# xiph/flac

Measured on NVIDIA H100. Metric: encode_msamples_per_s, higher is better.
Workload: dtype int32

## Files before the change

### flac_b200/csrc/autoc_kernel.cuh

```cuda
#pragma once

#include "device_common.cuh"

namespace fb200 {

__device__ __forceinline__ void cp_async_16(void *smem, const void *gmem)
{
	const unsigned s = (unsigned)__cvta_generic_to_shared(smem);
	asm volatile("cp.async.cg.shared.global [%0], [%1], 16;\n" ::"r"(s), "l"(gmem) : "memory");
}
__device__ __forceinline__ void cp_async_4_zfill(void *smem, const void *gmem, int src_bytes)
{
	const unsigned s = (unsigned)__cvta_generic_to_shared(smem);
	asm volatile("cp.async.ca.shared.global [%0], [%1], 4, %2;\n" ::"r"(s), "l"(gmem), "r"(src_bytes) : "memory");
}
__device__ __forceinline__ void cp_async_commit() { asm volatile("cp.async.commit_group;\n" ::: "memory"); }
template <int N>
__device__ __forceinline__ void cp_async_wait() { asm volatile("cp.async.wait_group %0;\n" ::"n"(N) : "memory"); }

__host__ __device__ constexpr int autoc3_stride(int T) { return ((T / 4) % 2 == 1) ? T : T + 4; }
template <int LAGS, int U, int K, int STAGES>
constexpr size_t autoc3_smem_bytes() { return (size_t)STAGES * (32 * autoc3_stride(U * K) + U * K) * 4; }

template <int LAGS, int U, int K, int STAGES>
__global__ void __launch_bounds__(32) k_autoc3(EncK P, const int32_t *__restrict__ sig, const SigMeta *__restrict__ meta,
                                              const float *__restrict__ windows, const DevSection *__restrict__ secs,
                                              double *__restrict__ autoc, int nitems)
{
	static_assert(U % LAGS == 0 && U % 4 == 0, "a body must be a whole number of history rotations and of 128-bit loads");
	constexpr int T = U * K;
	constexpr int STRIDE = autoc3_stride(T);
	constexpr int STAGE_WORDS = 32 * STRIDE + T;
	extern __shared__ int4 autoc3_smem[];
	int *const smem = reinterpret_cast<int *>(autoc3_smem);

	const int lane = threadIdx.x;
	const int groups = (nitems + 31) >> 5;
	const int sec = blockIdx.x / groups;
	const int item0 = (blockIdx.x - sec * groups) << 5;
	const int item = item0 + lane;
	const bool live = item < nitems && meta[min(item, nitems - 1)].bps != 0;
	if(!__any_sync(0xffffffffu, live)) return;

	const DevSection S = secs[sec];
	const float *w = windows + S.win_off;
	const int shift = S.partial ? S.data_shift : 0;
	const int a0 = shift & ~3;
	const int nvalid = S.partial ? 2 * S.part_size : S.data_len;
	const int wsecond = P.bs - 2 * S.part_size;
	const int ntiles = (shift - a0 + nvalid + T - 1) / T;

	auto issue = [&](int t) {
		if(t < ntiles) {
			int *st = smem + (t % STAGES) * STAGE_WORDS;
			const int32_t *g0 = sig + a0 + t * T;
#pragma unroll
			for(int j = 0; j < T / 4; j++) {
				const int idx = j * 32 + lane;
				const int row = idx / (T / 4), c = idx - row * (T / 4);
				cp_async_16(st + row * STRIDE + c * 4, g0 + (size_t)min(item0 + row, nitems - 1) * P.bs_stride + c * 4);
			}
#pragma unroll
			for(int j = 0; j < (T + 31) / 32; j++) {
				const int u = j * 32 + lane;
				if(u < T) {
					const int i = a0 + t * T + u - shift;
					const bool ok = i >= 0 && i < nvalid;
					const int wi = (!S.partial || i < S.part_size) ? i : wsecond + i;
					cp_async_4_zfill(st + 32 * STRIDE + u, ok ? (w + wi) : w, ok ? 4 : 0);
				}
			}
		}
		cp_async_commit();
	};

	double acc[LAGS], h[LAGS];
#pragma unroll
	for(int l = 0; l < LAGS; l++) { acc[l] = 0.0; h[l] = 0.0; }

#pragma unroll
	for(int t = 0; t < STAGES - 1; t++) issue(t);
	for(int t = 0; t < ntiles; t++) {
		cp_async_wait<STAGES - 2>();
		__syncwarp();
		issue(t + STAGES - 1);
		const int *row = smem + (t % STAGES) * STAGE_WORDS + lane * STRIDE;
		const float *win = reinterpret_cast<const float *>(smem + (t % STAGES) * STAGE_WORDS + 32 * STRIDE);
#pragma unroll 1
		for(int kb = 0; kb < K; kb++) {
#pragma unroll
			for(int q = 0; q < U / 4; q++) {
				const int4 xq = *reinterpret_cast<const int4 *>(row + kb * U + q * 4);
				const float4 wq = *reinterpret_cast<const float4 *>(win + kb * U + q * 4);
				const int xs[4] = {xq.x, xq.y, xq.z, xq.w};
				const float ws[4] = {wq.x, wq.y, wq.z, wq.w};
#pragma unroll
				for(int e = 0; e < 4; e++) {
					const int u = q * 4 + e;
					const double dv = (double)__fmul_rn((float)xs[e], ws[e]);
					const int su = (LAGS - (u % LAGS)) % LAGS;
					h[su] = dv;
#pragma unroll
					for(int l = 0; l < LAGS; l++) acc[l] = fma(dv, h[(su + l) % LAGS], acc[l]);
				}
			}
		}
	}
	if(live) {
		double *out = autoc + ((size_t)sec * nitems + item) * P.lag_stride;
#pragma unroll
		for(int l = 0; l < LAGS; l++) out[l] = acc[l];
	}
}


__host__ __device__ constexpr int autoc4_rows_max(int nsig) { return (nsig + 30) / nsig + 1; }
__host__ __device__ constexpr int autoc4_row_stride(int T, int ch, int mode)
{
	return mode == 2 ? T * ch + 8 : (((T * ch / 4) & 1) ? T * ch : T * ch + 4);
}
template <int U, int K, int STAGES>
__host__ __device__ constexpr size_t autoc4_smem_bytes(int nsig, int ch, int mode)
{
	return 64 + (size_t)STAGES * ((size_t)autoc4_rows_max(nsig) * autoc4_row_stride(U * K, ch, mode) + U * K) * 4;
}

template <int LAGS, int U, int K, int STAGES, int MODE>
__global__ void __launch_bounds__(32) k_autoc4(EncK P, const int32_t *__restrict__ pcm, const SigMeta *__restrict__ meta,
                                              const float *__restrict__ secwin, int secwin_stride, const DevSection *__restrict__ secs,
                                              double *__restrict__ autoc, int nitems, uint32_t *__restrict__ sigor, int or_sec)
{
	static_assert(U % LAGS == 0 && U % 4 == 0, "a body must be a whole number of history rotations and of 128-bit loads");
	constexpr int T = U * K;
	extern __shared__ int4 autoc4_smem[];
	uint64_t *const bars = reinterpret_cast<uint64_t *>(autoc4_smem);
	int *const smem = reinterpret_cast<int *>(autoc4_smem) + 16;
	const int lane = threadIdx.x, nsig = P.nsig, ch = P.channels, bs = P.bs;
	const int RS = autoc4_row_stride(T, ch, MODE);
	const int STAGE_WORDS = autoc4_rows_max(nsig) * RS + T;

	const int groups = (nitems + 31) >> 5;
	const int sec = blockIdx.x / groups;
	const bool do_or = sigor != nullptr && sec == or_sec;
	uint32_t orv = 0;
	const int item0 = (blockIdx.x - sec * groups) << 5;
	const int item = min(item0 + lane, nitems - 1);
	SigMeta M;
	M.wasted = 0; M.bps = 1;
	if(meta) M = meta[item];
	const bool live = item0 + lane < nitems && M.bps != 0;
	if(!__any_sync(0xffffffffu, live)) return;

	const DevSection S = secs[sec];
	const int shift = S.partial ? S.data_shift : 0;
	const int a0 = shift & ~3;
	const int nvalid = S.partial ? 2 * S.part_size : S.data_len;
	const int ntiles = (shift - a0 + nvalid + T - 1) / T;
	const int b0 = item0 / nsig;
	const int nrows = min(item0 + 31, nitems - 1) / nsig - b0 + 1;
	const int myrow = item / nsig - b0, sidx = item - (item / nsig) * nsig;
	const float *wsec = secwin + (size_t)sec * secwin_stride;

	int ca = 1, cb = 0, sh = M.wasted;
	if(MODE == 1) {
		if(sidx == 1) { ca = 0; cb = 1; }
		else if(sidx == 2) { ca = 1; cb = 1; sh += 1; }
		else if(sidx == 3) { ca = 1; cb = -1; }
	}

	if(lane == 0) {
#pragma unroll
		for(int s = 0; s < STAGES; s++) mbar_init(&bars[s], 1);
		mbar_fence_init();
	}
	__syncwarp();

	auto issue = [&](int t) {
		if(t < ntiles) {
			const int stg = t % STAGES;
			int *st = smem + stg * STAGE_WORDS;
			const int start = a0 + t * T;
			const int n = min(T, bs - start);
			const unsigned row_bytes = (unsigned)n * (unsigned)ch * 4u;
			if(lane == 0) mbar_expect_tx(&bars[stg], (unsigned)nrows * row_bytes + (unsigned)T * 4u);
			__syncwarp();
			if(lane < nrows) tma_bulk_g2s(st + lane * RS, pcm + ((size_t)(b0 + lane) * bs + start) * ch, row_bytes, &bars[stg]);
			if(lane == (nrows < 32 ? nrows : 0)) tma_bulk_g2s(st + autoc4_rows_max(nsig) * RS, wsec + start, (unsigned)T * 4u, &bars[stg]);
		}
	};

	double acc[LAGS], h[LAGS];
#pragma unroll
	for(int l = 0; l < LAGS; l++) { acc[l] = 0.0; h[l] = 0.0; }

#pragma unroll
	for(int t = 0; t < STAGES - 1; t++) issue(t);
	for(int t = 0; t < ntiles; t++) {
		__syncwarp();
		issue(t + STAGES - 1);
		mbar_wait(&bars[t % STAGES], (unsigned)(t / STAGES) & 1u);
		if(do_or && bs - (a0 + t * T) < T) {
			const int n = bs - (a0 + t * T);
			int *st = smem + (t % STAGES) * STAGE_WORDS;
			for(int r = 0; r < nrows; r++)
				for(int i = n * ch + lane; i < T * ch; i += 32) st[r * RS + i] = 0;
			__syncwarp();
		}
		const int *row = smem + (t % STAGES) * STAGE_WORDS + myrow * RS;
		const float *win = reinterpret_cast<const float *>(smem + (t % STAGES) * STAGE_WORDS + autoc4_rows_max(nsig) * RS);
#pragma unroll 1
		for(int kb = 0; kb < K; kb++) {
#pragma unroll
			for(int q = 0; q < U / 4; q++) {
				int xs4[4];
				if(MODE == 0) {
					const int4 xq = *reinterpret_cast<const int4 *>(row + kb * U + q * 4);
					xs4[0] = xq.x >> sh; xs4[1] = xq.y >> sh; xs4[2] = xq.z >> sh; xs4[3] = xq.w >> sh;
				}
				else if(MODE == 1) {
					const int4 p0 = *reinterpret_cast<const int4 *>(row + 2 * (kb * U + q * 4));
					const int4 p1 = *reinterpret_cast<const int4 *>(row + 2 * (kb * U + q * 4) + 4);
					xs4[0] = (ca * p0.x + cb * p0.y) >> sh; xs4[1] = (ca * p0.z + cb * p0.w) >> sh;
					xs4[2] = (ca * p1.x + cb * p1.y) >> sh; xs4[3] = (ca * p1.z + cb * p1.w) >> sh;
				}
				else {
#pragma unroll
					for(int e = 0; e < 4; e++) xs4[e] = row[(kb * U + q * 4 + e) * ch + sidx] >> sh;
				}
				const float4 wq = *reinterpret_cast<const float4 *>(win + kb * U + q * 4);
				const float ws[4] = {wq.x, wq.y, wq.z, wq.w};
				orv |= (uint32_t)(xs4[0] | xs4[1]) | (uint32_t)(xs4[2] | xs4[3]);
#pragma unroll
				for(int e = 0; e < 4; e++) {
					const int u = q * 4 + e;
					const double dv = (double)__fmul_rn((float)xs4[e], ws[e]);
					const int su = (LAGS - (u % LAGS)) % LAGS;
					h[su] = dv;
#pragma unroll
					for(int l = 0; l < LAGS; l++) acc[l] = fma(dv, h[(su + l) % LAGS], acc[l]);
				}
			}
		}
	}
	if(live) {
		double *out = autoc + ((size_t)sec * nitems + item) * P.lag_stride;
#pragma unroll
		for(int l = 0; l < LAGS; l++) out[l] = acc[l];
		if(do_or) sigor[item] = orv;
	}
}

}
```

### flac_b200/csrc/search_kernel.cuh

```cuda
#pragma once

#include "device_common.cuh"

namespace fb200 {

template <int G, int MAXORD, int NTAPS, bool MASKED>
__device__ __forceinline__ void group_abs_sum_f64(const int (&xg)[MAXORD + G], const double (&qd)[MAXORD], int ord0, int limit, double &sd, bool &bad)
{
	constexpr double kFloorMagic = 6755399441055744.0;
	double xd[MAXORD + G];
#pragma unroll
	for(int i = MAXORD - NTAPS; i < MAXORD + G; i++) xd[i] = int_to_double_exact(xg[i]);
#pragma unroll
	for(int m = 0; m < G; m++) {
		double sum = 0.0;
#pragma unroll
		for(int j = 0; j < NTAPS; j++) sum = fma(qd[j], xd[MAXORD + m - 1 - j], sum);
		const double t = __dadd_rd(sum, kFloorMagic);
		const double rr = __dadd_rn(__dsub_rn(xd[MAXORD + m], t), kFloorMagic);
		if(limit && (rr <= -2147483648.0 || rr > 2147483647.0)) bad = true;
		bool keep = true;
		if(MASKED && m < MAXORD) keep = m >= ord0;
		if(keep) sd = __dadd_rn(sd, fabs(rr));
	}
}

template <int R_T, int MAXORD, int NTAPS, bool WIDE, bool NARROW>
__device__ __forceinline__ bool fir_partition_sums(const int32_t *xs, const int (&q)[MAXORD], int shift, int order, int limit,
                                                   int ntiles, int lane, int lpp_log, int tpp, bool mask32, unsigned long long *leaf)
{
	constexpr int G = (R_T == 32) ? 16 : 12, NG = R_T / G, ROWPAD = 36 - R_T;
	bool bad = false;
	unsigned long long carry = 0;
	double qd[MAXORD];
	if(WIDE) {
		const double scale = __hiloint2double((1023 - shift) << 20, 0);
#pragma unroll
		for(int j = 0; j < MAXORD; j++) qd[j] = __dmul_rn((double)q[j], scale);
	}
	unsigned long long warm = 0;
	{
		int xw[MAXORD];
#pragma unroll
		for(int k = 0; k < MAXORD / 4; k++) {
			const int4 v = *reinterpret_cast<const int4 *>(xs + 4 * k);
			xw[4 * k] = v.x; xw[4 * k + 1] = v.y; xw[4 * k + 2] = v.z; xw[4 * k + 3] = v.w;
		}
#pragma unroll
		for(int m = 0; m < MAXORD; m++) {
			unsigned long long a;
			if(!WIDE) {
				int sum = 0;
#pragma unroll
				for(int j = 0; j < (m < NTAPS ? m : NTAPS); j++) sum += q[j] * xw[m - 1 - j];
				a = __sad(xw[m], sum >> shift, 0u);
			}
			else {
				long long sum = 0;
#pragma unroll
				for(int j = 0; j < (m < NTAPS ? m : NTAPS); j++) sum += (long long)q[j] * (long long)xw[m - 1 - j];
				const long long rr = (long long)xw[m] - (sum >> shift);
				a = (unsigned long long)(rr < 0 ? -rr : rr);
			}
			if(m < order) warm += a;
		}
	}
#pragma unroll 1
	for(int t = 0; t < ntiles; t++) {
		const int32_t *rowp = xs + (t * 32 + lane) * 36;
		uint32_t s32 = 0;
		unsigned long long s64 = 0;
		double sd = 0.0;
#pragma unroll 1
		for(int g = 0; g < NG; g++) {
			int xg[MAXORD + G];
			const int32_t *op = rowp + g * G;
#pragma unroll
			for(int k = 0; k < MAXORD / 4; k++) {
				const int4 v = *reinterpret_cast<const int4 *>(op - MAXORD + 4 * k - ((g * G + 4 * k < MAXORD) ? ROWPAD : 0));
				xg[4 * k] = v.x; xg[4 * k + 1] = v.y; xg[4 * k + 2] = v.z; xg[4 * k + 3] = v.w;
			}
#pragma unroll
			for(int k = 0; k < G / 4; k++) {
				const int4 v = *reinterpret_cast<const int4 *>(op + 4 * k);
				xg[MAXORD + 4 * k] = v.x; xg[MAXORD + 4 * k + 1] = v.y; xg[MAXORD + 4 * k + 2] = v.z; xg[MAXORD + 4 * k + 3] = v.w;
			}
			if(WIDE) group_abs_sum_f64<G, MAXORD, NTAPS, false>(xg, qd, 0, limit, sd, bad);
			else group_abs_sum<G, MAXORD, NTAPS, false, false, NARROW>(xg, q, shift, 0, limit, s32, s64, bad);
		}
		if(WIDE) s64 = (unsigned long long)__double2ll_rn(sd);
		if(tpp == 1) {
			const int lpp = 1 << lpp_log;
			if(NARROW) {
				uint32_t s = s32;
				for(int o = lpp >> 1; o > 0; o >>= 1) s += __shfl_xor_sync(0xffffffffu, s, o);
				if(t == 0 && lane == 0) s -= (uint32_t)warm;
				if((lane & (lpp - 1)) == 0) leaf[(t * 32 + lane) >> lpp_log] = s;
			}
			else {
				unsigned long long s = s64;
				for(int o = lpp >> 1; o > 0; o >>= 1) s += __shfl_xor_sync(0xffffffffu, s, o);
				if(t == 0 && lane == 0) s -= warm;
				if((lane & (lpp - 1)) == 0) leaf[(t * 32 + lane) >> lpp_log] = mask32 ? (unsigned long long)(uint32_t)s : s;
			}
		}
		else {
			carry += warp_sum_u64(NARROW ? (unsigned long long)s32 : s64);
			if(t + 1 == tpp) carry -= warm;
			if((t + 1) % tpp == 0) {
				if(lane == 0) leaf[t / tpp] = (NARROW || mask32) ? (unsigned long long)(uint32_t)carry : carry;
				carry = 0;
			}
		}
	}
	return bad;
}

struct SearchResult5 {
	uint32_t best_bits;
	int idx, type, order, prec, shift, method, po, wide, pad;
	int q[FB200_MAX_LPC_ORDER];
};

__host__ __device__ constexpr size_t search5_scratch_bytes(int max_po)
{
	return (((size_t)8 << max_po) + ((size_t)3 << max_po) + 15) / 16 * 16;
}
__host__ __device__ constexpr size_t search5_smem_bytes(int bs, int R_T, int nsig, int wps, int max_po)
{
	return (size_t)nsig * (size_t)(kSearch4ZeroRow + (bs / R_T) * 36) * 4 + (size_t)nsig * wps * search5_scratch_bytes(max_po) +
	       (size_t)nsig * (sizeof(SearchResult5) + 16) + 64 + (size_t)nsig * 48;
}

template <int R_T, int MAXORD, int WPS, bool WIDEK>
__global__ void __launch_bounds__(256, 2) k_search5(EncK P, const int32_t *__restrict__ pcm, const SigMeta *__restrict__ meta,
                                                    const CandDesc *__restrict__ cdesc, SubframePlan *__restrict__ plans)
{
	static_assert(MAXORD >= 8 && MAXORD % 4 == 0 && R_T % 4 == 0 && MAXORD + 4 <= kSearch4ZeroRow, "vector loads / zero row");
	extern __shared__ __align__(16) unsigned char smem_raw[];
	const int tid = threadIdx.x, NT = blockDim.x, warp = tid >> 5, lane = tid & 31, bs = P.bs, ch = P.channels;
	const int ngroups = P.sig_group ? (P.nsig + P.sig_group - 1) / P.sig_group : 1;
	const int blk = (int)blockIdx.x / ngroups;
	const int sig0 = P.sig_group ? ((int)blockIdx.x - blk * ngroups) * P.sig_group : 0;
	const int nsig = P.sig_group ? min(P.sig_group, P.nsig - sig0) : P.nsig;
	if(P.redo && !P.redo[blk]) return;
	const int nrows = bs / R_T;
	const int slice_words = kSearch4ZeroRow + nrows * 36;
	int32_t *const slices = reinterpret_cast<int32_t *>(smem_raw);
	unsigned char *const scratch0 = smem_raw + (size_t)nsig * slice_words * 4;
	const size_t scratch_bytes = search5_scratch_bytes(P.max_po);
	unsigned char *const after_scratch = scratch0 + (size_t)nsig * WPS * scratch_bytes;
	SearchResult5 *const results = reinterpret_cast<SearchResult5 *>(after_scratch);
	int *const queues = reinterpret_cast<int *>(after_scratch + (size_t)nsig * sizeof(SearchResult5));
	uint64_t *const mbar = reinterpret_cast<uint64_t *>(queues + nsig + (nsig & 1));
	unsigned long long *const xch_all = reinterpret_cast<unsigned long long *>(mbar + 1);

	const SigMeta *bm = meta + (size_t)blk * P.nsig + sig0;
	const bool stereo_ms = (ch == 2 && P.nsig == 4);

	if(tid < nsig) queues[tid] = 0;
	const int32_t *graw = pcm + (size_t)blk * bs * ch;
	if(ch <= 2 && (bs * ch) % (4 * NT) == 0 && (bs * ch / 4) / NT <= 16) {
		const unsigned raw_bytes = (unsigned)bs * (unsigned)ch * 4u;
		int32_t *const raw = slices + kSearch4ZeroRow + ((nsig * slice_words - kSearch4ZeroRow - bs * ch) & ~3);
		if(tid == 0) {
			mbar_init(mbar, 1);
			mbar_fence_init();
			mbar_expect_tx(mbar, raw_bytes);
			tma_bulk_g2s(raw, graw, raw_bytes, mbar);
		}
		__syncthreads();
		mbar_wait(mbar, 0);
		int4 rv[16];
		const int nv = (bs * ch / 4) / NT;
#pragma unroll
		for(int k = 0; k < 16; k++)
			if(k < nv) rv[k] = *reinterpret_cast<const int4 *>(raw + 4 * (k * NT + tid));
		__syncthreads();
		for(int s = warp; s < nsig; s += NT >> 5)
			for(int i = lane; i < kSearch4ZeroRow; i += 32) slices[s * slice_words + i] = 0;
		if(ch == 2) {
			const int w0 = bm[0].wasted, w1 = bm[1].wasted;
			const int w2 = stereo_ms ? bm[2].wasted : 0, w3 = stereo_ms ? bm[3].wasted : 0;
			int32_t *const p0 = slices + kSearch4ZeroRow, *const p1 = p0 + slice_words, *const p2 = p1 + slice_words, *const p3 = p2 + slice_words;
#pragma unroll
			for(int k = 0; k < 16; k++)
				if(k < nv) {
					const int i = 2 * (k * NT + tid);
					const int row = i / R_T, off = row * 36 + (i - row * R_T);
					const int L0 = rv[k].x, R0 = rv[k].y, L1 = rv[k].z, R1 = rv[k].w;
					*reinterpret_cast<int2 *>(p0 + off) = make_int2(L0 >> w0, L1 >> w0);
					*reinterpret_cast<int2 *>(p1 + off) = make_int2(R0 >> w1, R1 >> w1);
					if(stereo_ms) {
						*reinterpret_cast<int2 *>(p2 + off) = make_int2(((L0 + R0) >> 1) >> w2, ((L1 + R1) >> 1) >> w2);
						*reinterpret_cast<int2 *>(p3 + off) = make_int2((L0 - R0) >> w3, (L1 - R1) >> w3);
					}
				}
		}
		else {
			const int w0 = bm[0].wasted;
			int32_t *const p0 = slices + kSearch4ZeroRow;
#pragma unroll
			for(int k = 0; k < 16; k++)
				if(k < nv) {
					const int i = 4 * (k * NT + tid);
					const int row = i / R_T, off = row * 36 + (i - row * R_T);
					*reinterpret_cast<int4 *>(p0 + off) = make_int4(rv[k].x >> w0, rv[k].y >> w0, rv[k].z >> w0, rv[k].w >> w0);
				}
		}
	}
	else {
		for(int s = warp; s < nsig; s += NT >> 5) {
			const int w = bm[s].wasted;
			int32_t *const ps = slices + s * slice_words + kSearch4ZeroRow;
			for(int i = lane; i < kSearch4ZeroRow; i += 32) ps[i - kSearch4ZeroRow] = 0;
			for(int i = lane; i < bs; i += 32) {
				int v;
				if(stereo_ms && s >= 2) {
					const int L = __ldg(graw + 2 * i), R = __ldg(graw + 2 * i + 1);
					v = s == 2 ? ((L + R) >> 1) : (L - R);
				}
				else v = __ldg(graw + (size_t)i * ch + sig0 + s);
				const int row = i / R_T;
				ps[row * 36 + (i - row * R_T)] = v >> w;
			}
		}
	}
	__syncthreads();

	const int sidx = warp / WPS, part = warp - sidx * WPS;
	const bool have_signal = sidx < nsig;
	const bool skip_sig = P.redo != nullptr && sig0 + sidx < ch - 1;
	const SigMeta M = have_signal ? bm[sidx] : SigMeta{0, 0};
	const bool active = have_signal && M.bps != 0 && !skip_sig;
	const int32_t *const xs = slices + (have_signal ? sidx : 0) * slice_words + kSearch4ZeroRow;
	unsigned char *const my_scratch = scratch0 + (size_t)(have_signal ? warp : 0) * scratch_bytes;
	unsigned long long *const leaf = reinterpret_cast<unsigned long long *>(my_scratch);
	uint8_t *const params_all = my_scratch + ((size_t)8 << P.max_po);
	uint8_t *const b_params = params_all + ((size_t)2 << P.max_po);
	const int sbps = M.bps, wasted = M.wasted;

	constexpr int TILE = 32 * R_T;
	constexpr int GAPV = (R_T == 32 ? 4 : 0) / 4;
	const int ntiles = bs / TILE;

	uint32_t best_bits = 0xffffffffu;
	int b_idx = -1, b_type = SF_VERBATIM, b_order = 0, b_prec = 0, b_shift = 0, b_method = 0, b_po = 0, b_wide = 0;
	int b_q[MAXORD];
#pragma unroll
	for(int j = 0; j < MAXORD; j++) b_q[j] = 0;
	bool is_constant = false;

	if(active) {
		for(int p = lane; p < (1 << P.max_po); p += 32) b_params[p] = 0;
		if(!(P.dis_verb && bs >= (int)kMaxFixedOrder)) best_bits = kSubframeHeaderBits + (uint32_t)wasted + (uint32_t)bs * (uint32_t)sbps;
		__syncwarp();

		auto evaluate = [&](int cand_index, int type, int order, int precision, int shift, int wide, int limit, const int (&q)[MAXORD]) {
			int max_po = P.max_po;
			while(max_po > 0 && (bs >> max_po) <= order) max_po--;
			const int min_po = min(P.min_po, max_po);
			const int psize = bs >> max_po;
			const bool narrow = (uint32_t)(sbps + (int)kMaxExtraResidualBps) < 32u - ilog2_u32((uint32_t)psize);
			const int tpp = psize > TILE ? psize / TILE : 1;
			const int lpp_log = tpp == 1 ? (int)ilog2_u32((uint32_t)(psize / R_T)) : 5;

			constexpr int NT12 = MAXORD < 12 ? MAXORD : 12;
			bool bad = false;
			const bool via_f64 = wide || (WIDEK && WPS == 2 && part == 1 && P.f64b != 0);
			if(!via_f64 && narrow) {
				if(order <= 4) bad = fir_partition_sums<R_T, MAXORD, 4, false, true>(xs, q, shift, order, 0, ntiles, lane, lpp_log, tpp, true, leaf);
				else if(order <= 8) bad = fir_partition_sums<R_T, MAXORD, 8, false, true>(xs, q, shift, order, 0, ntiles, lane, lpp_log, tpp, true, leaf);
				else if(MAXORD > 8 && order <= 12) bad = fir_partition_sums<R_T, MAXORD, NT12, false, true>(xs, q, shift, order, 0, ntiles, lane, lpp_log, tpp, true, leaf);
				else bad = fir_partition_sums<R_T, MAXORD, MAXORD, false, true>(xs, q, shift, order, 0, ntiles, lane, lpp_log, tpp, true, leaf);
			}
			else if(!via_f64) {
				if(order <= 8) bad = fir_partition_sums<R_T, MAXORD, 8, false, false>(xs, q, shift, order, 0, ntiles, lane, lpp_log, tpp, narrow, leaf);
				else if(MAXORD > 8 && order <= 12) bad = fir_partition_sums<R_T, MAXORD, NT12, false, false>(xs, q, shift, order, 0, ntiles, lane, lpp_log, tpp, narrow, leaf);
				else bad = fir_partition_sums<R_T, MAXORD, MAXORD, false, false>(xs, q, shift, order, 0, ntiles, lane, lpp_log, tpp, narrow, leaf);
			}
			else if(WIDEK) {
				if(order <= 8) bad = fir_partition_sums<R_T, MAXORD, 8, true, false>(xs, q, shift, order, limit, ntiles, lane, lpp_log, tpp, narrow, leaf);
				else if(MAXORD > 8 && order <= 12) bad = fir_partition_sums<R_T, MAXORD, NT12, true, false>(xs, q, shift, order, limit, ntiles, lane, lpp_log, tpp, narrow, leaf);
				else bad = fir_partition_sums<R_T, MAXORD, MAXORD, true, false>(xs, q, shift, order, limit, ntiles, lane, lpp_log, tpp, narrow, leaf);
			}
			else bad = fir_partition_sums<R_T, MAXORD, MAXORD, true, false>(xs, q, shift, order, limit, ntiles, lane, lpp_log, tpp, narrow, leaf);
			if(__any_sync(0xffffffffu, bad)) return;
			__syncwarp();

			uint32_t best_r = 0;
			int best_po = 0;
			const uint32_t rice_cap = (uint32_t)P.rice_limit - 1;
			auto node_bits = [&](unsigned long long mean, uint32_t psamp, uint32_t div, int n, bool own) -> uint32_t {
				uint32_t k;
				if((mean >> 32) == 0) {
					const uint32_t m32 = (uint32_t)mean;
					const uint32_t m1 = m32 - 1;
					const uint32_t t = m32 < 2 ? 0u : __funnelshift_r(m1 * div, __umulhi(m1, div), 18);
					k = t ? 32u - (uint32_t)__clz((int)t) : 0u;
				}
				else {
					const unsigned long long t = ((mean - 1) * div) >> 18;
					k = t ? ilog2_u64(t) + 1 : 0u;
				}
				if(k > rice_cap) k = rice_cap;
				if(own) params_all[n] = (uint8_t)k;
				return own ? count_rice_bits(k, psamp, mean) : 0u;
			};
			auto close_order = [&](int po, unsigned long long lane_bits) {
				unsigned long long total;
				if(__any_sync(0xffffffffu, (lane_bits >> 27) != 0)) total = warp_sum_u64(lane_bits);
				else total = __reduce_add_sync(0xffffffffu, (unsigned)lane_bits);
				total += kEntropyTypeLen + kRiceOrderLen;
				const uint32_t bits = (uint32_t)(total < 0xffffffffull ? total : 0xffffffffull);
				if(best_r == 0 || bits < best_r) { best_r = bits; best_po = po; }
			};
			unsigned long long cur;
			int lev;
			if(max_po >= 5) {
				unsigned long long v[8];
				const int cnt0 = 1 << (max_po - 5);
	#pragma unroll
				for(int i = 0; i < 8; i++) v[i] = i < cnt0 ? leaf[lane * cnt0 + i] : 0ull;
				int po = max_po;
	#pragma unroll 1
				for(; po >= 5 && po >= min_po; po--) {
					const int cnt = 1 << (po - 5);
					const uint32_t pbase = (uint32_t)(bs >> po);
					const uint32_t div_rest = 0x40000u / pbase, div_first = 0x40000u / (pbase - (uint32_t)order);
					unsigned long long b = 0;
	#pragma unroll
					for(int i = 0; i < 8; i++)
						if(i < cnt) {
							const int p = lane * cnt + i;
							b += node_bits(v[i], p == 0 ? pbase - (uint32_t)order : pbase, p == 0 ? div_first : div_rest, (1 << po) + p, true);
						}
					close_order(po, b);
	#pragma unroll
					for(int i = 0; i < 4; i++)
						if(2 * i + 1 < cnt) v[i] = v[2 * i] + v[2 * i + 1];
				}
				cur = v[0];
				lev = 5;
			}
			else {
				cur = leaf[lane >> (5 - max_po)];
				lev = max_po;
			}
			if(min_po <= 4) {
				const int n1 = lane + 1;
				const int myL = (int)ilog2_u32((uint32_t)n1);
				const int myP = n1 - (1 << myL);
				unsigned long long mine = 0;
	#pragma unroll 1
				for(int L = 4; L >= 0; L--) {
					if(L < lev) cur += __shfl_xor_sync(0xffffffffu, cur, 16 >> L);
					const unsigned long long got = __shfl_sync(0xffffffffu, cur, (myP << (5 - L)) & 31);
					if(myL == L) mine = got;
				}
				const int top = max_po < 4 ? max_po : 4;
				const bool active = lane < 31 && myL >= min_po && myL <= top;
				const uint32_t psamp = (uint32_t)(bs >> myL) - (myP == 0 ? (uint32_t)order : 0u);
				const uint32_t bits = node_bits(mine, psamp, 0x40000u / psamp, n1, active);
	#pragma unroll 1
				for(int L = top; L >= min_po; L--)
					if(true) close_order(L, (active && myL == L) ? bits : 0u);
			}

			uint32_t estimate = kSubframeHeaderBits + (uint32_t)wasted;
			if(type == SF_FIXED) estimate += (uint32_t)order * (uint32_t)sbps;
			else estimate += kQlpPrecisionLen + kQlpShiftLen + (uint32_t)order * (uint32_t)(precision + sbps);
			if(best_r < 0xffffffffu - estimate) estimate += best_r;
			else estimate = 0xffffffffu;
			const bool better = (type == SF_LPC ? estimate > 0 : true) && estimate < best_bits;
			if(better) {
				__syncwarp();
				uint32_t any15 = 0;
				for(int p = lane; p < (1 << best_po); p += 32) {
					const uint8_t k = params_all[(1 << best_po) + p];
					b_params[p] = k;
					any15 |= (k >= kRiceEscape) ? 1u : 0u;
				}
				any15 = warp_or(any15);
				best_bits = estimate;
				b_idx = cand_index;
				b_type = type; b_order = order; b_prec = precision; b_shift = shift; b_method = any15 ? 1 : 0; b_po = best_po; b_wide = wide;
	#pragma unroll
				for(int j = 0; j < MAXORD; j++) b_q[j] = (type == SF_LPC) ? q[j] : 0;
			}
			__syncwarp();
		};


		if(bs > (int)kMaxFixedOrder) {
			if(part == 0 || WPS == 2) {
				unsigned long long te[5] = {0, 0, 0, 0, 0};
				uint32_t diff = 0;
				const int32_t x0 = xs[0];
				const bool lane_total_fits = (uint32_t)(sbps + 3) + ilog2_u32((uint32_t)(2 * (bs / 32) - 1)) <= 32u;
				uint32_t t32[5] = {0, 0, 0, 0, 0};
		#pragma unroll 1
				for(int t = (WPS == 2 ? part : 0); t < ntiles; t += WPS) {
					const int row = t * 32 + lane;
					int xw[4 + R_T];
					{
						const int4 *pv = reinterpret_cast<const int4 *>(xs + row * 36);
						const int4 hv = pv[-1 - GAPV];
						xw[0] = hv.x; xw[1] = hv.y; xw[2] = hv.z; xw[3] = hv.w;
		#pragma unroll
						for(int k = 0; k < R_T / 4; k++) {
							const int4 v = pv[k];
							xw[4 + 4 * k] = v.x; xw[5 + 4 * k] = v.y; xw[6 + 4 * k] = v.z; xw[7 + 4 * k] = v.w;
						}
					}
					int e1[R_T + 3], e2[R_T + 2], e3[R_T + 1];
		#pragma unroll
					for(int k = 0; k < R_T + 3; k++) e1[k] = xw[k + 1] - xw[k];
		#pragma unroll
					for(int k = 0; k < R_T + 2; k++) e2[k] = e1[k + 1] - e1[k];
		#pragma unroll
					for(int k = 0; k < R_T + 1; k++) e3[k] = e2[k + 1] - e2[k];
		#pragma unroll
					for(int m = 0; m < R_T; m++) {
						diff |= (uint32_t)(xw[4 + m] ^ x0);
						const bool counted = m >= (int)kMaxFixedOrder || row != 0;
						if(counted) {
							t32[0] = __sad(xw[4 + m], 0, t32[0]);
							t32[1] = __sad(e1[m + 3], 0, t32[1]);
							t32[2] = __sad(e2[m + 2], 0, t32[2]);
							t32[3] = __sad(e3[m + 1], 0, t32[3]);
							t32[4] = __sad(e3[m + 1] - e3[m], 0, t32[4]);
						}
						if((m & 3) == 3 && !lane_total_fits) {
		#pragma unroll
							for(int k = 0; k < 5; k++) { te[k] += t32[k]; t32[k] = 0; }
						}
					}
				}
		#pragma unroll
				for(int k = 0; k < 5; k++) te[k] += t32[k];
				uint32_t eq = diff == 0 ? 1u : 0u;
		#pragma unroll
				for(int k = 0; k < 5; k++) te[k] = warp_sum_u64(te[k]);
				eq = warp_and(eq);
				if(WPS == 2) {
					unsigned long long *xch = xch_all + 6 * sidx;
					if(part == 1) {
						if(lane == 0) {
#pragma unroll
							for(int k = 0; k < 5; k++) xch[k] = te[k];
							xch[5] = eq;
						}
						__threadfence_block();
						asm volatile("bar.arrive %0, 64;" ::"r"(1 + sidx) : "memory");
					}
					else {
						asm volatile("bar.sync %0, 64;" ::"r"(1 + sidx) : "memory");
#pragma unroll
						for(int k = 0; k < 5; k++) te[k] += xch[k];
						eq &= (uint32_t)xch[5];
					}
				}
				if(part == 0) {
				int guess;
				{
					const unsigned long long m34 = te[3] < te[4] ? te[3] : te[4], m234 = te[2] < m34 ? te[2] : m34, m1234 = te[1] < m234 ? te[1] : m234;
					if(te[0] <= m1234) guess = 0;
					else if(te[1] <= m234) guess = 1;
					else if(te[2] <= m34) guess = 2;
					else if(te[3] <= te[4]) guess = 3;
					else guess = 4;
				}
				float rbps[5];
				{
					const double n = (double)(uint32_t)(bs - (int)kMaxFixedOrder);
					unsigned long long mine = te[0];
		#pragma unroll
					for(int k = 1; k < 5; k++) mine = lane == k ? te[k] : mine;
					const float r = (float)((mine > 0) ? fb_log(M_LN2 * (double)mine / n) / M_LN2 : 0.0);
		#pragma unroll
					for(int k = 0; k < 5; k++) rbps[k] = __shfl_sync(0xffffffffu, r, k);
				}
				is_constant = !P.dis_const && rbps[1] == 0.0f && eq;
				if(is_constant) {
					const uint32_t cbits = kSubframeHeaderBits + (uint32_t)wasted + (uint32_t)sbps;
					if(cbits < best_bits) { best_bits = cbits; b_type = SF_CONSTANT; b_idx = 0; }
				}
				else if(!P.dis_fixed || (P.max_order == 0 && best_bits == 0xffffffffu)) {
					int lo, hi;
					if(P.exhaustive) { lo = 0; hi = (int)kMaxFixedOrder; }
					else lo = hi = guess;
					if(hi >= bs) hi = bs - 1;
					for(int fo = lo; fo <= hi; fo++) {
						if(rbps[fo] >= (float)sbps) continue;
						int q[MAXORD];
#pragma unroll
						for(int j = 0; j < MAXORD; j++) q[j] = fixed_tap(fo, j);
						evaluate(fo, SF_FIXED, fo, 0, 0, 0, 0, q);
					}
				}
				}
			}
			if(P.max_order > 0 && !is_constant) {
				const CandDesc *cd = cdesc + ((size_t)blk * P.nsig + sig0 + sidx) * P.nslots;
				for(;;) {
					int c = 0;
					if(lane == 0) c = atomicAdd(&queues[sidx], 1);
					c = __shfl_sync(0xffffffffu, c, 0);
					if(c >= P.nslots) break;
					const CandDesc *D = cd + c;
					if(!__ldg(&D->valid)) continue;
					int q[MAXORD];
#pragma unroll
					for(int j = 0; j < MAXORD; j++) q[j] = __ldg(&D->qlp[j]);
					evaluate(5 + c, SF_LPC, __ldg(&D->order), __ldg(&D->precision), __ldg(&D->shift), __ldg(&D->wide), __ldg(&D->limit), q);
				}
			}
		}
	}

	if(WPS > 1 && active && part != 0 && lane == 0) {
		SearchResult5 &Rz = results[sidx];
		Rz.best_bits = best_bits; Rz.idx = b_idx; Rz.type = b_type; Rz.order = b_order; Rz.prec = b_prec; Rz.shift = b_shift;
		Rz.method = b_method; Rz.po = b_po; Rz.wide = b_wide;
#pragma unroll
		for(int j = 0; j < MAXORD; j++) Rz.q[j] = b_q[j];
	}
	__syncthreads();
	if(!have_signal || part != 0 || skip_sig) return;
	SubframePlan *plan = plans + (size_t)blk * P.nsig + sig0 + sidx;
	if(!active) {
		if(lane == 0) { plan->type = -1; plan->est_bits = 0xffffffffu; }
		return;
	}
	const uint8_t *win_params = b_params;
	if(WPS > 1 && !is_constant) {
		const SearchResult5 &Rz = results[sidx];
		const bool other = Rz.best_bits < best_bits || (Rz.best_bits == best_bits && Rz.idx >= 0 && (b_idx < 0 ? false : Rz.idx < b_idx));
		if(other) {
			best_bits = Rz.best_bits; b_type = Rz.type; b_order = Rz.order; b_prec = Rz.prec; b_shift = Rz.shift; b_method = Rz.method; b_po = Rz.po; b_wide = Rz.wide;
#pragma unroll
			for(int j = 0; j < MAXORD; j++) b_q[j] = Rz.q[j];
			win_params = scratch0 + (size_t)(warp + 1) * scratch_bytes + ((size_t)8 << P.max_po) + ((size_t)2 << P.max_po);
		}
	}
	if(best_bits == 0xffffffffu) {
		b_type = SF_VERBATIM;
		best_bits = kSubframeHeaderBits + (uint32_t)wasted + (uint32_t)bs * (uint32_t)sbps;
	}
	if(lane == 0) {
		plan->type = b_type; plan->order = b_order; plan->wasted = wasted; plan->bps = sbps;
		plan->precision = b_prec; plan->shift = b_shift; plan->method = b_method; plan->porder = b_po;
		plan->est_bits = best_bits; plan->wide = b_wide;
#pragma unroll
		for(int j = 0; j < FB200_MAX_LPC_ORDER; j++) plan->qlp[j] = (j < MAXORD) ? b_q[j < MAXORD ? j : 0] : 0;
	}
	for(int p = lane; p < kMaxPartitions; p += 32) plan->params[p] = p < (1 << P.max_po) ? win_params[p] : 0;
}

}
```

Before: 66320.

## Reuse fixed-predictor partition sums and split single LPC candidate across warp pair

The fixed-order residual pass now stores per-partition absolute-residual leaves in shared memory, so fixed orders are evaluated from those leaves instead of rerunning the FIR partition-sum pass. When a signal has fewer LPC candidates than warps, the two warps split the LPC tile range and sync through named barriers, with the part-1 warp finishing the evaluation. This adds shared memory, extra barriers and reordered phases in exchange for less redundant residual computation and better warp utilisation. The autocorrelation smem row count is also tightened when nsig divides 32.

```diff
diff --git a/flac_b200/csrc/autoc_kernel.cuh b/flac_b200/csrc/autoc_kernel.cuh
--- a/flac_b200/csrc/autoc_kernel.cuh
+++ b/flac_b200/csrc/autoc_kernel.cuh
@@ -114,7 +114,7 @@
 }
 
 
-__host__ __device__ constexpr int autoc4_rows_max(int nsig) { return (nsig + 30) / nsig + 1; }
+__host__ __device__ constexpr int autoc4_rows_max(int nsig) { return 32 % nsig == 0 ? 32 / nsig : (nsig + 30) / nsig + 1; }
 __host__ __device__ constexpr int autoc4_row_stride(int T, int ch, int mode)
 {
 	return mode == 2 ? T * ch + 8 : (((T * ch / 4) & 1) ? T * ch : T * ch + 4);
diff --git a/flac_b200/csrc/search_kernel.cuh b/flac_b200/csrc/search_kernel.cuh
--- a/flac_b200/csrc/search_kernel.cuh
+++ b/flac_b200/csrc/search_kernel.cuh
@@ -27,7 +27,8 @@
 
 template <int R_T, int MAXORD, int NTAPS, bool WIDE, bool NARROW>
 __device__ __forceinline__ bool fir_partition_sums(const int32_t *xs, const int (&q)[MAXORD], int shift, int order, int limit,
-                                                   int ntiles, int lane, int lpp_log, int tpp, bool mask32, unsigned long long *leaf)
+                                                   int t0, int tstep, int ntiles, int lane, int lpp_log, int tpp, bool mask32,
+                                                   unsigned long long *leaf)
 {
 	constexpr int G = (R_T == 32) ? 16 : 12, NG = R_T / G, ROWPAD = 36 - R_T;
 	bool bad = false;
@@ -39,7 +40,7 @@
 		for(int j = 0; j < MAXORD; j++) qd[j] = __dmul_rn((double)q[j], scale);
 	}
 	unsigned long long warm = 0;
-	{
+	if(t0 == 0) {
 		int xw[MAXORD];
 #pragma unroll
 		for(int k = 0; k < MAXORD / 4; k++) {
@@ -66,7 +67,7 @@
 		}
 	}
 #pragma unroll 1
-	for(int t = 0; t < ntiles; t++) {
+	for(int t = t0; t < ntiles; t += tstep) {
 		const int32_t *rowp = xs + (t * 32 + lane) * 36;
 		uint32_t s32 = 0;
 		unsigned long long s64 = 0;
@@ -126,10 +127,18 @@
 {
 	return (((size_t)8 << max_po) + ((size_t)3 << max_po) + 15) / 16 * 16;
 }
+__host__ __device__ constexpr int search5_fixed_leaves(int bs, int R_T, int max_po)
+{
+	return (1 << max_po) > bs / (32 * R_T) ? (1 << max_po) : bs / (32 * R_T);
+}
+__host__ __device__ constexpr size_t search5_fixed_bytes(int bs, int R_T, int max_po)
+{
+	return ((size_t)5 * 8 * search5_fixed_leaves(bs, R_T, max_po) + 15) / 16 * 16;
+}
 __host__ __device__ constexpr size_t search5_smem_bytes(int bs, int R_T, int nsig, int wps, int max_po)
 {
 	return (size_t)nsig * (size_t)(kSearch4ZeroRow + (bs / R_T) * 36) * 4 + (size_t)nsig * wps * search5_scratch_bytes(max_po) +
-	       (size_t)nsig * (sizeof(SearchResult5) + 16) + 64 + (size_t)nsig * 48;
+	       (size_t)nsig * search5_fixed_bytes(bs, R_T, max_po) + (size_t)nsig * (sizeof(SearchResult5) + 16) + 64 + (size_t)nsig * wps * 64;
 }
 
 template <int R_T, int MAXORD, int WPS, bool WIDEK>
@@ -149,7 +158,9 @@
 	int32_t *const slices = reinterpret_cast<int32_t *>(smem_raw);
 	unsigned char *const scratch0 = smem_raw + (size_t)nsig * slice_words * 4;
 	const size_t scratch_bytes = search5_scratch_bytes(P.max_po);
-	unsigned char *const after_scratch = scratch0 + (size_t)nsig * WPS * scratch_bytes;
+	unsigned char *const fixed0 = scratch0 + (size_t)nsig * WPS * scratch_bytes;
+	const size_t fixed_bytes = search5_fixed_bytes(bs, R_T, P.max_po);
+	unsigned char *const after_scratch = fixed0 + (size_t)nsig * fixed_bytes;
 	SearchResult5 *const results = reinterpret_cast<SearchResult5 *>(after_scratch);
 	int *const queues = reinterpret_cast<int *>(after_scratch + (size_t)nsig * sizeof(SearchResult5));
 	uint64_t *const mbar = reinterpret_cast<uint64_t *>(queues + nsig + (nsig & 1));
@@ -243,6 +254,13 @@
 	constexpr int TILE = 32 * R_T;
 	constexpr int GAPV = (R_T == 32 ? 4 : 0) / 4;
 	const int ntiles = bs / TILE;
+	const bool split = WPS == 2 && P.nslots < WPS;
+	unsigned long long *const lpc_leaf =
+		split ? reinterpret_cast<unsigned long long *>(scratch0 + (size_t)((have_signal ? sidx : 0) * WPS + WPS - 1) * scratch_bytes) : leaf;
+	unsigned long long *const fleaf = reinterpret_cast<unsigned long long *>(fixed0 + (size_t)(have_signal ? sidx : 0) * fixed_bytes);
+	const int psize_fx = bs >> P.max_po;
+	const int lpp_log_fx = psize_fx > TILE ? 5 : (int)ilog2_u32((uint32_t)(psize_fx / R_T));
+	const int nleaf_fx = search5_fixed_leaves(bs, R_T, P.max_po);
 
 	uint32_t best_bits = 0xffffffffu;
 	int b_idx = -1, b_type = SF_VERBATIM, b_order = 0, b_prec = 0, b_shift = 0, b_method = 0, b_po = 0, b_wide = 0;
@@ -256,37 +274,48 @@
 		if(!(P.dis_verb && bs >= (int)kMaxFixedOrder)) best_bits = kSubframeHeaderBits + (uint32_t)wasted + (uint32_t)bs * (uint32_t)sbps;
 		__syncwarp();
 
-		auto evaluate = [&](int cand_index, int type, int order, int precision, int shift, int wide, int limit, const int (&q)[MAXORD]) {
-			int max_po = P.max_po;
-			while(max_po > 0 && (bs >> max_po) <= order) max_po--;
-			const int min_po = min(P.min_po, max_po);
-			const int psize = bs >> max_po;
-			const bool narrow = (uint32_t)(sbps + (int)kMaxExtraResidualBps) < 32u - ilog2_u32((uint32_t)psize);
-			const int tpp = psize > TILE ? psize / TILE : 1;
-			const int lpp_log = tpp == 1 ? (int)ilog2_u32((uint32_t)(psize / R_T)) : 5;
-
+		struct Geo { int max_po, min_po, tpp, lpp_log; bool narrow; };
+		auto geometry = [&](int order) {
+			Geo g;
+			g.max_po = P.max_po;
+			while(g.max_po > 0 && (bs >> g.max_po) <= order) g.max_po--;
+			g.min_po = min(P.min_po, g.max_po);
+			const int psize = bs >> g.max_po;
+			g.narrow = (uint32_t)(sbps + (int)kMaxExtraResidualBps) < 32u - ilog2_u32((uint32_t)psize);
+			g.tpp = psize > TILE ? psize / TILE : 1;
+			g.lpp_log = g.tpp == 1 ? (int)ilog2_u32((uint32_t)(psize / R_T)) : 5;
+			return g;
+		};
+
+		auto lpc_pass = [&](const Geo &g, int order, int shift, int wide, int limit, const int (&q)[MAXORD], int t0, int tstep, unsigned long long *lf) -> bool {
 			constexpr int NT12 = MAXORD < 12 ? MAXORD : 12;
+			const int tpp = g.tpp, lpp_log = g.lpp_log;
+			const bool narrow = g.narrow;
 			bool bad = false;
 			const bool via_f64 = wide || (WIDEK && WPS == 2 && part == 1 && P.f64b != 0);
 			if(!via_f64 && narrow) {
-				if(order <= 4) bad = fir_partition_sums<R_T, MAXORD, 4, false, true>(xs, q, shift, order, 0, ntiles, lane, lpp_log, tpp, true, leaf);
-				else if(order <= 8) bad = fir_partition_sums<R_T, MAXORD, 8, false, true>(xs, q, shift, order, 0, ntiles, lane, lpp_log, tpp, true, leaf);
-				else if(MAXORD > 8 && order <= 12) bad = fir_partition_sums<R_T, MAXORD, NT12, false, true>(xs, q, shift, order, 0, ntiles, lane, lpp_log, tpp, true, leaf);
-				else bad = fir_partition_sums<R_T, MAXORD, MAXORD, false, true>(xs, q, shift, order, 0, ntiles, lane, lpp_log, tpp, true, leaf);
+				if(order <= 4) bad = fir_partition_sums<R_T, MAXORD, 4, false, true>(xs, q, shift, order, 0, t0, tstep, ntiles, lane, lpp_log, tpp, true, lf);
+				else if(order <= 8) bad = fir_partition_sums<R_T, MAXORD, 8, false, true>(xs, q, shift, order, 0, t0, tstep, ntiles, lane, lpp_log, tpp, true, lf);
+				else if(MAXORD > 8 && order <= 12) bad = fir_partition_sums<R_T, MAXORD, NT12, false, true>(xs, q, shift, order, 0, t0, tstep, ntiles, lane, lpp_log, tpp, true, lf);
+				else bad = fir_partition_sums<R_T, MAXORD, MAXORD, false, true>(xs, q, shift, order, 0, t0, tstep, ntiles, lane, lpp_log, tpp, true, lf);
 			}
 			else if(!via_f64) {
-				if(order <= 8) bad = fir_partition_sums<R_T, MAXORD, 8, false, false>(xs, q, shift, order, 0, ntiles, lane, lpp_log, tpp, narrow, leaf);
-				else if(MAXORD > 8 && order <= 12) bad = fir_partition_sums<R_T, MAXORD, NT12, false, false>(xs, q, shift, order, 0, ntiles, lane, lpp_log, tpp, narrow, leaf);
-				else bad = fir_partition_sums<R_T, MAXORD, MAXORD, false, false>(xs, q, shift, order, 0, ntiles, lane, lpp_log, tpp, narrow, leaf);
+				if(order <= 8) bad = fir_partition_sums<R_T, MAXORD, 8, false, false>(xs, q, shift, order, 0, t0, tstep, ntiles, lane, lpp_log, tpp, narrow, lf);
+				else if(MAXORD > 8 && order <= 12) bad = fir_partition_sums<R_T, MAXORD, NT12, false, false>(xs, q, shift, order, 0, t0, tstep, ntiles, lane, lpp_log, tpp, narrow, lf);
+				else bad = fir_partition_sums<R_T, MAXORD, MAXORD, false, false>(xs, q, shift, order, 0, t0, tstep, ntiles, lane, lpp_log, tpp, narrow, lf);
 			}
 			else if(WIDEK) {
-				if(order <= 8) bad = fir_partition_sums<R_T, MAXORD, 8, true, false>(xs, q, shift, order, limit, ntiles, lane, lpp_log, tpp, narrow, leaf);
-				else if(MAXORD > 8 && order <= 12) bad = fir_partition_sums<R_T, MAXORD, NT12, true, false>(xs, q, shift, order, limit, ntiles, lane, lpp_log, tpp, narrow, leaf);
-				else bad = fir_partition_sums<R_T, MAXORD, MAXORD, true, false>(xs, q, shift, order, limit, ntiles, lane, lpp_log, tpp, narrow, leaf);
-			}
-			else bad = fir_partition_sums<R_T, MAXORD, MAXORD, true, false>(xs, q, shift, order, limit, ntiles, lane, lpp_log, tpp, narrow, leaf);
-			if(__any_sync(0xffffffffu, bad)) return;
-			__syncwarp();
+				if(order <= 8) bad = fir_partition_sums<R_T, MAXORD, 8, true, false>(xs, q, shift, order, limit, t0, tstep, ntiles, lane, lpp_log, tpp, narrow, lf);
+				else if(MAXORD > 8 && order <= 12) bad = fir_partition_sums<R_T, MAXORD, NT12, true, false>(xs, q, shift, order, limit, t0, tstep, ntiles, lane, lpp_log, tpp, narrow, lf);
+				else bad = fir_partition_sums<R_T, MAXORD, MAXORD, true, false>(xs, q, shift, order, limit, t0, tstep, ntiles, lane, lpp_log, tpp, narrow, lf);
+			}
+			else bad = fir_partition_sums<R_T, MAXORD, MAXORD, true, false>(xs, q, shift, order, limit, t0, tstep, ntiles, lane, lpp_log, tpp, narrow, lf);
+			return bad;
+		};
+
+		auto evaluate = [&](const Geo &g, int cand_index, int type, int order, int precision, int shift, int wide, const int (&q)[MAXORD],
+		                    const unsigned long long *lf) {
+			const int max_po = g.max_po, min_po = g.min_po;
 
 			uint32_t best_r = 0;
 			int best_po = 0;
@@ -321,7 +350,7 @@
 				unsigned long long v[8];
 				const int cnt0 = 1 << (max_po - 5);
 	#pragma unroll
-				for(int i = 0; i < 8; i++) v[i] = i < cnt0 ? leaf[lane * cnt0 + i] : 0ull;
+				for(int i = 0; i < 8; i++) v[i] = i < cnt0 ? lf[lane * cnt0 + i] : 0ull;
 				int po = max_po;
 	#pragma unroll 1
 				for(; po >= 5 && po >= min_po; po--) {
@@ -344,7 +373,7 @@
 				lev = 5;
 			}
 			else {
-				cur = leaf[lane >> (5 - max_po)];
+				cur = lf[lane >> (5 - max_po)];
 				lev = max_po;
 			}
 			if(min_po <= 4) {
@@ -398,7 +427,6 @@
 				uint32_t diff = 0;
 				const int32_t x0 = xs[0];
 				const bool lane_total_fits = (uint32_t)(sbps + 3) + ilog2_u32((uint32_t)(2 * (bs / 32) - 1)) <= 32u;
-				uint32_t t32[5] = {0, 0, 0, 0, 0};
 		#pragma unroll 1
 				for(int t = (WPS == 2 ? part : 0); t < ntiles; t += WPS) {
 					const int row = t * 32 + lane;
@@ -420,6 +448,9 @@
 					for(int k = 0; k < R_T + 2; k++) e2[k] = e1[k + 1] - e1[k];
 		#pragma unroll
 					for(int k = 0; k < R_T + 1; k++) e3[k] = e2[k + 1] - e2[k];
+					uint32_t t32[5] = {0, 0, 0, 0, 0};
+					unsigned long long r64[5] = {0, 0, 0, 0, 0};
+					uint32_t w32[4] = {0, 0, 0, 0};
 		#pragma unroll
 					for(int m = 0; m < R_T; m++) {
 						diff |= (uint32_t)(xw[4 + m] ^ x0);
@@ -431,89 +462,149 @@
 							t32[3] = __sad(e3[m + 1], 0, t32[3]);
 							t32[4] = __sad(e3[m + 1] - e3[m], 0, t32[4]);
 						}
+						else {
+							w32[0] = __sad(xw[4 + m], 0, w32[0]);
+							if(m >= 1) w32[1] = __sad(e1[m + 3], 0, w32[1]);
+							if(m >= 2) w32[2] = __sad(e2[m + 2], 0, w32[2]);
+							if(m >= 3) w32[3] = __sad(e3[m + 1], 0, w32[3]);
+						}
 						if((m & 3) == 3 && !lane_total_fits) {
 		#pragma unroll
-							for(int k = 0; k < 5; k++) { te[k] += t32[k]; t32[k] = 0; }
-						}
-					}
-				}
-		#pragma unroll
-				for(int k = 0; k < 5; k++) te[k] += t32[k];
+							for(int k = 0; k < 5; k++) { r64[k] += t32[k]; t32[k] = 0; }
+						}
+					}
+					const int lpp = 1 << lpp_log_fx;
+		#pragma unroll
+					for(int k = 0; k < 5; k++) {
+						r64[k] += t32[k];
+						te[k] += r64[k];
+						if(k < 4) r64[k] += w32[k < 4 ? k : 0];
+					}
+		#pragma unroll 1
+					for(int o = 1; o < lpp; o <<= 1) {
+		#pragma unroll
+						for(int k = 0; k < 5; k++) r64[k] += __shfl_xor_sync(0xffffffffu, r64[k], o);
+					}
+					if((lane & (lpp - 1)) == 0) {
+		#pragma unroll
+						for(int k = 0; k < 5; k++) fleaf[k * nleaf_fx + (row >> lpp_log_fx)] = r64[k];
+					}
+				}
+				__syncwarp();
 				uint32_t eq = diff == 0 ? 1u : 0u;
 		#pragma unroll
 				for(int k = 0; k < 5; k++) te[k] = warp_sum_u64(te[k]);
 				eq = warp_and(eq);
-				if(WPS == 2) {
-					unsigned long long *xch = xch_all + 6 * sidx;
-					if(part == 1) {
-						if(lane == 0) {
-#pragma unroll
-							for(int k = 0; k < 5; k++) xch[k] = te[k];
-							xch[5] = eq;
-						}
-						__threadfence_block();
-						asm volatile("bar.arrive %0, 64;" ::"r"(1 + sidx) : "memory");
+				if(lane == 0) {
+					unsigned long long *xch = xch_all + 8 * warp;
+#pragma unroll
+					for(int k = 0; k < 5; k++) xch[k] = te[k];
+					xch[5] = eq;
+				}
+				if(WPS == 2 && part == 1) {
+					__threadfence_block();
+					asm volatile("bar.arrive %0, 64;" ::"r"(1 + sidx) : "memory");
+				}
+			}
+			for(int phase = 0; phase < 2; phase++) {
+				if((phase == 0) != split) {
+					if(part != 0) continue;
+					uint32_t fix_orders = 0;
+					{
+						const unsigned long long *xch = xch_all + 8 * warp;
+						if(WPS == 2) asm volatile("bar.sync %0, 64;" ::"r"(1 + sidx) : "memory");
+						else __syncwarp();
+						unsigned long long te[5];
+#pragma unroll
+						for(int k = 0; k < 5; k++) te[k] = xch[k] + (WPS == 2 ? xch[8 + k] : 0ull);
+						const uint32_t eq = (uint32_t)xch[5] & (WPS == 2 ? (uint32_t)xch[13] : 1u);
+						int guess;
+						{
+							const unsigned long long m34 = te[3] < te[4] ? te[3] : te[4], m234 = te[2] < m34 ? te[2] : m34, m1234 = te[1] < m234 ? te[1] : m234;
+							if(te[0] <= m1234) guess = 0;
+							else if(te[1] <= m234) guess = 1;
+							else if(te[2] <= m34) guess = 2;
+							else if(te[3] <= te[4]) guess = 3;
+							else guess = 4;
+						}
+						float rbps[5];
+						{
+							const double n = (double)(uint32_t)(bs - (int)kMaxFixedOrder);
+							unsigned long long mine = te[0];
+#pragma unroll
+							for(int k = 1; k < 5; k++) mine = lane == k ? te[k] : mine;
+							const float r = (float)((mine > 0) ? fb_log(M_LN2 * (double)mine / n) / M_LN2 : 0.0);
+#pragma unroll
+							for(int k = 0; k < 5; k++) rbps[k] = __shfl_sync(0xffffffffu, r, k);
+						}
+						is_constant = !P.dis_const && rbps[1] == 0.0f && eq;
+						if(is_constant) {
+							const uint32_t cbits = kSubframeHeaderBits + (uint32_t)wasted + (uint32_t)sbps;
+							if(cbits < best_bits) { best_bits = cbits; b_type = SF_CONSTANT; b_idx = 0; }
+						}
+						else if(!P.dis_fixed || (P.max_order == 0 && best_bits == 0xffffffffu)) {
+							int lo, hi;
+							if(P.exhaustive) { lo = 0; hi = (int)kMaxFixedOrder; }
+							else lo = hi = guess;
+							if(hi >= bs) hi = bs - 1;
+							for(int fo = lo; fo <= hi; fo++)
+								if(rbps[fo] < (float)sbps) fix_orders |= 1u << fo;
+						}
+					}
+					int qz[MAXORD];
+#pragma unroll
+					for(int j = 0; j < MAXORD; j++) qz[j] = 0;
+					for(int fo = 0; fo <= (int)kMaxFixedOrder; fo++) {
+						if(!((fix_orders >> fo) & 1u)) continue;
+						const Geo g = geometry(fo);
+						for(int p = lane; p < (1 << g.max_po); p += 32) {
+							unsigned long long s = 0;
+							for(int j = 0; j < g.tpp; j++) s += fleaf[fo * nleaf_fx + p * g.tpp + j];
+							leaf[p] = g.narrow ? (unsigned long long)(uint32_t)s : s;
+						}
+						__syncwarp();
+						evaluate(g, fo, SF_FIXED, fo, 0, 0, 0, qz, leaf);
+					}
+					continue;
+				}
+				if(!(P.max_order > 0 && (split || !is_constant))) continue;
+				const CandDesc *cd = cdesc + ((size_t)blk * P.nsig + sig0 + sidx) * P.nslots;
+				for(int it = 0;; it++) {
+					int c = 0;
+					if(split) {
+						if(it) break;
 					}
 					else {
-						asm volatile("bar.sync %0, 64;" ::"r"(1 + sidx) : "memory");
-#pragma unroll
-						for(int k = 0; k < 5; k++) te[k] += xch[k];
-						eq &= (uint32_t)xch[5];
-					}
-				}
-				if(part == 0) {
-				int guess;
-				{
-					const unsigned long long m34 = te[3] < te[4] ? te[3] : te[4], m234 = te[2] < m34 ? te[2] : m34, m1234 = te[1] < m234 ? te[1] : m234;
-					if(te[0] <= m1234) guess = 0;
-					else if(te[1] <= m234) guess = 1;
-					else if(te[2] <= m34) guess = 2;
-					else if(te[3] <= te[4]) guess = 3;
-					else guess = 4;
-				}
-				float rbps[5];
-				{
-					const double n = (double)(uint32_t)(bs - (int)kMaxFixedOrder);
-					unsigned long long mine = te[0];
-		#pragma unroll
-					for(int k = 1; k < 5; k++) mine = lane == k ? te[k] : mine;
-					const float r = (float)((mine > 0) ? fb_log(M_LN2 * (double)mine / n) / M_LN2 : 0.0);
-		#pragma unroll
-					for(int k = 0; k < 5; k++) rbps[k] = __shfl_sync(0xffffffffu, r, k);
-				}
-				is_constant = !P.dis_const && rbps[1] == 0.0f && eq;
-				if(is_constant) {
-					const uint32_t cbits = kSubframeHeaderBits + (uint32_t)wasted + (uint32_t)sbps;
-					if(cbits < best_bits) { best_bits = cbits; b_type = SF_CONSTANT; b_idx = 0; }
-				}
-				else if(!P.dis_fixed || (P.max_order == 0 && best_bits == 0xffffffffu)) {
-					int lo, hi;
-					if(P.exhaustive) { lo = 0; hi = (int)kMaxFixedOrder; }
-					else lo = hi = guess;
-					if(hi >= bs) hi = bs - 1;
-					for(int fo = lo; fo <= hi; fo++) {
-						if(rbps[fo] >= (float)sbps) continue;
-						int q[MAXORD];
-#pragma unroll
-						for(int j = 0; j < MAXORD; j++) q[j] = fixed_tap(fo, j);
-						evaluate(fo, SF_FIXED, fo, 0, 0, 0, 0, q);
-					}
-				}
-				}
-			}
-			if(P.max_order > 0 && !is_constant) {
-				const CandDesc *cd = cdesc + ((size_t)blk * P.nsig + sig0 + sidx) * P.nslots;
-				for(;;) {
-					int c = 0;
-					if(lane == 0) c = atomicAdd(&queues[sidx], 1);
-					c = __shfl_sync(0xffffffffu, c, 0);
+						if(lane == 0) c = atomicAdd(&queues[sidx], 1);
+						c = __shfl_sync(0xffffffffu, c, 0);
+					}
 					if(c >= P.nslots) break;
 					const CandDesc *D = cd + c;
 					if(!__ldg(&D->valid)) continue;
 					int q[MAXORD];
 #pragma unroll
 					for(int j = 0; j < MAXORD; j++) q[j] = __ldg(&D->qlp[j]);
-					evaluate(5 + c, SF_LPC, __ldg(&D->order), __ldg(&D->precision), __ldg(&D->shift), __ldg(&D->wide), __ldg(&D->limit), q);
+					const int order = __ldg(&D->order), shift = __ldg(&D->shift), wide = __ldg(&D->wide);
+					const Geo g = geometry(order);
+					const bool halves = split && g.tpp == 1 && ntiles > 1;
+					if(split && !halves && part == 0) break;
+					bool bad = false;
+					if(!is_constant) bad = lpc_pass(g, order, shift, wide, __ldg(&D->limit), q, halves ? part : 0, halves ? WPS : 1, lpc_leaf);
+					bool any_bad = __any_sync(0xffffffffu, bad);
+					if(halves) {
+						unsigned long long *xch = xch_all + 8 * (sidx * WPS);
+						if(part == 0) {
+							if(lane == 0) xch[6] = any_bad ? 1ull : 0ull;
+							__threadfence_block();
+							asm volatile("bar.arrive %0, 64;" ::"r"(5 + sidx) : "memory");
+							break;
+						}
+						asm volatile("bar.sync %0, 64;" ::"r"(5 + sidx) : "memory");
+						any_bad = any_bad || xch[6] != 0;
+					}
+					if(any_bad) continue;
+					__syncwarp();
+					evaluate(g, 5 + c, SF_LPC, order, __ldg(&D->precision), shift, wide, q, lpc_leaf);
 				}
 			}
 		}
```

New measurement: 67280 (median of 6 runs). 1.01x the previous value.
